# uncertaintyhub/chsimpy

Measured on AMD Instinct MI355X. Metric: timesteps/sec at N=4096 fp64; achieved HBM GB/s vs MI355X peak, higher is better.
Workload: dtype f64; 1 GPU; N=4096 fp64 Cahn-Hilliard timestep loop (BASELINE.json configs[2] at N=4096), U_init = 0.875 + 0.00875*(PCG64(2023).random - 0.5), kappa_tilde=0.0002989112919661156, full_sim; N=4096, engine=fast, ensemble=single run

## Files before the change

### chsimpy_amd/csrc/chs_fast_core.h

```cpp
#pragma once
#include <hip/hip_runtime.h>
#include <type_traits>
#include "chs_cx.h"

template <typename T_, int N_, int G_, int THREADS_, int R0_, int RA_, int RB_, int RL_, int PAD1_, int PAD2_,
          int PADL_, int WPS_, int CT_ = THREADS_ / G_, int XPAIR_ = -1>
struct FCfg {
  using T = T_;
  using V = Cx<T_>;
  static constexpr int N = N_;
  static constexpr int M = N_ / 2;
  static constexpr int G = G_;
  static constexpr int E = M / G_;
  static constexpr int R0 = R0_, RA = RA_, RB = RB_, RL = RL_;
  static constexpr int R2 = RL_;
  static constexpr int S1 = R0_;
  static constexpr int S2A = R0_ * RA_;
  static constexpr int SL = R0_ * RA_ * RB_;
  static constexpr int S2 = SL;
  static constexpr int L1 = M / R0_;
  static constexpr int L2 = L1 / RA_;
  static constexpr int L3 = L2 / RB_;
  static constexpr int NP0 = E / (2 * R0_);
  static constexpr int NBA = E / RA_;
// ... 19 lines not shown
  static_assert(NP0 >= 1 && NP2 >= 1, "E must be >= 2*R0 and >= 2*RL");
  static_assert(RA_ == 1 || NBA >= 1, "E must be >= RA");
  static_assert(RB_ == 1 || NBB >= 1, "E must be >= RB");
  static_assert((G_ <= 64 && (64 % G_) == 0) || (G_ % 64) == 0, "group size");
  static_assert(THREADS_ % G_ == 0 && THREADS_ % 64 == 0, "workgroup size");
};

template <typename T>
struct FTables {
  const T* tw0;
  const T* twa;
  const T* twb;
  const T* wp;
  const T* t1;
  const T* t2;
  const T* lam4;
  const T* sin4;
};

#define FC_SQRT1_2 0.70710678118654752440
#define FC_COS_PI_8 0.92387953251128675613
#define FC_SIN_PI_8 0.38268343236508977173

template <int IDX, bool CONJ>
struct W16 {
  static constexpr int idx = ((CONJ ? -IDX : IDX) % 16 + 16) % 16;
  static constexpr bool pure = (idx % 4) == 0;
};

template <class V, int IDX, bool CONJ>
__device__ __forceinline__ V mul_w16(V a) {
  constexpr int idx = W16<IDX, CONJ>::idx;
  using S = decltype(cx_re(a));
  const V one = cx_make(S(1), S(1));
  if constexpr (idx == 0) {
    return a;
  } else if constexpr (idx == 4) {
    return pk_mul_k<1, 0, 0, 1, 0, 1, 0, 0>(a, one);
  } else if constexpr (idx == 8) {
    return pk_mul_k<0, 1, 0, 1, 1, 1, 0, 0>(a, one);
  } else if constexpr (idx == 12) {
    return pk_mul_k<1, 0, 0, 1, 1, 0, 0, 0>(a, one);
  } else {
    constexpr double cs[16] = {1.0, FC_COS_PI_8, FC_SQRT1_2, FC_SIN_PI_8, 0.0, -FC_SIN_PI_8, -FC_SQRT1_2, -FC_COS_PI_8,
                               -1.0, -FC_COS_PI_8, -FC_SQRT1_2, -FC_SIN_PI_8, 0.0, FC_SIN_PI_8, FC_SQRT1_2, FC_COS_PI_8};
    constexpr double sn[16] = {0.0, FC_SIN_PI_8, FC_SQRT1_2, FC_COS_PI_8, 1.0, FC_COS_PI_8, FC_SQRT1_2, FC_SIN_PI_8,
                               0.0, -FC_SIN_PI_8, -FC_SQRT1_2, -FC_COS_PI_8, -1.0, -FC_COS_PI_8, -FC_SQRT1_2, -FC_SIN_PI_8};
    return cx_mul_k(a, cx_make((S)cs[idx], (S)-sn[idx]));
  }
}

template <class V, int ROT>
__device__ __forceinline__ void bfly2_rot(V& a, V& b) {
  static_assert(ROT % 4 == 0, "pure rotations only");
  constexpr int r = ((ROT % 16) + 16) % 16;
  const V x = a, y = b;
  if constexpr (r == 0) { a = cx_add(x, y); b = cx_sub(x, y); }
  else if constexpr (r == 4) { a = cx_add_mi(x, y); b = cx_add_pi(x, y); }
  else if constexpr (r == 8) { a = cx_sub(x, y); b = cx_add(x, y); }
  else { a = cx_add_pi(x, y); b = cx_add_mi(x, y); }
}

template <class V, int R, bool INV>
struct Dft;

template <class V, bool INV>
struct Dft<V, 1, INV> {
  static __device__ __forceinline__ void run(V*) {}
};

template <class V, bool INV>
struct Dft<V, 2, INV> {
  static __device__ __forceinline__ void run(V* z) { bfly2_rot<V, 0>(z[0], z[1]); }
};

template <class V, bool INV>
struct Dft<V, 4, INV> {
  static __device__ __forceinline__ void run(V* z) {
    const V t0 = cx_add(z[0], z[2]), t1 = cx_sub(z[0], z[2]);
    const V t2 = cx_add(z[1], z[3]), t3 = cx_sub(z[1], z[3]);
    z[0] = cx_add(t0, t2);
    z[2] = cx_sub(t0, t2);
    if constexpr (!INV) { z[1] = cx_add_mi(t1, t3); z[3] = cx_add_pi(t1, t3); }
    else { z[1] = cx_add_pi(t1, t3); z[3] = cx_add_mi(t1, t3); }
  }
};

template <class V, int R, bool INV>
struct Dft {
  static constexpr int A = 4, B = R / 4;
  static_assert(R == 8 || R == 16, "radix must be 2, 4, 8 or 16");
  template <int N2, int K1>
  static constexpr int tw_idx() { return (N2 * K1 * 16) / R; }
  template <int N2, int K1>
  static __device__ __forceinline__ V tw(V a) {
    if constexpr (B == 2 && W16<tw_idx<N2, K1>(), INV>::pure) return a;
    else return mul_w16<V, tw_idx<N2, K1>(), INV>(a);
  }
  template <int N2>
  static __device__ __forceinline__ void col(const V* z, V (*c)[A]) {
    V x[A];
#pragma unroll
    for (int n1 = 0; n1 < A; ++n1) x[n1] = z[B * n1 + N2];
    Dft<V, A, INV>::run(x);
    c[N2][0] = x[0];
    c[N2][1] = tw<N2, 1>(x[1]);
    c[N2][2] = tw<N2, 2>(x[2]);
    c[N2][3] = tw<N2, 3>(x[3]);
  }
  template <int K1>
  static __device__ __forceinline__ void row(V* z, V (*c)[A]) {
    if constexpr (B == 2) {
      V y0 = c[0][K1], y1 = c[1][K1];
      constexpr int rot = W16<tw_idx<1, K1>(), INV>::pure ? W16<tw_idx<1, K1>(), INV>::idx : 0;
      bfly2_rot<V, rot>(y0, y1);
      z[K1] = y0; z[K1 + A] = y1;
    } else {
      V y[B];
#pragma unroll
      for (int n2 = 0; n2 < B; ++n2) y[n2] = c[n2][K1];
      Dft<V, B, INV>::run(y);
#pragma unroll
      for (int k2 = 0; k2 < B; ++k2) z[K1 + A * k2] = y[k2];
    }
  }
  static __device__ __forceinline__ void run(V* z) {
    V c[B][A];
    col<0>(z, c);
    col<1>(z, c);
    if constexpr (B == 4) {
      col<2>(z, c);
      col<3>(z, c);
    }
    row<0>(z, c);
    row<1>(z, c);
    row<2>(z, c);
    row<3>(z, c);
  }
};

template <typename T>
__device__ __forceinline__ Cx<T> ldc(const T* __restrict__ tab, int idx) {
  if constexpr (sizeof(T) == 8) {
    const double2 v = *reinterpret_cast<const double2*>(tab + 2 * (size_t)idx);
    return cx_make(v.x, v.y);
  } else {
    return *reinterpret_cast<const v2f*>(tab + 2 * (size_t)idx);
  }
}

typedef double chs_dv2 __attribute__((ext_vector_type(2)));
template <typename T, bool NT>
__device__ __forceinline__ Cx<T> ldc_hint(const T* __restrict__ tab, int idx) {
  if constexpr (!NT) {
    return ldc<T>(tab, idx);
  } else if constexpr (sizeof(T) == 8) {
    const chs_dv2 v = __builtin_nontemporal_load(reinterpret_cast<const chs_dv2*>(tab + 2 * (size_t)idx));
    return cx_make(v.x, v.y);
  } else {
    return __builtin_nontemporal_load(reinterpret_cast<const v2f*>(tab + 2 * (size_t)idx));
  }
}

template <class C>
__device__ __forceinline__ void xsync() {
  if constexpr (C::WAVE_LOCAL) {
    __builtin_amdgcn_fence(__ATOMIC_RELEASE, "wavefront");
    __builtin_amdgcn_wave_barrier();
    __builtin_amdgcn_fence(__ATOMIC_ACQUIRE, "wavefront");
  } else {
    __syncthreads();
  }
}

// ... 480 lines not shown
```

### chsimpy_amd/csrc/chs_fast_kernels.h

```cpp
#pragma once
#include <cmath>
#include <vector>
#include <cstdlib>

#include "chs_common.h"
#ifdef CHS_STAMPS
#define CHS_NSTAMP 12
#ifdef CHS_FAST_MAIN_TU
__device__ unsigned long long g_stamps[2][8192 * CHS_NSTAMP];
#endif
#define STAMP(K, I)                                                                         \
  do {                                                                                      \
    __builtin_amdgcn_sched_barrier(0);                                                      \
    unsigned long long t__;                                                                 \
    asm volatile("s_memtime %0\n\ts_waitcnt lgkmcnt(0)" : "=s"(t__)::"memory");            \
    __builtin_amdgcn_sched_barrier(0);                                                      \
    if (threadIdx.x == 0 && blockIdx.x < 8192) g_stamps[K][blockIdx.x * CHS_NSTAMP + (I)] = t__; \
  } while (0)
#define CHS_RSTAMP(I) do { if constexpr (PIPE) STAMP(1, 6 + (I)); } while (0)
#define CHS_RSTAMP1(I)                                                                      \
  do {                                                                                      \
    if constexpr (PIPE) {                                                                   \
      __builtin_amdgcn_sched_barrier(0);                                                    \
      unsigned long long t__;                                                               \
// ... 259 lines not shown
  T* ltw = reinterpret_cast<T*>(chs_dyn_lds + (size_t)C::C * C::SCR * sizeof(T) + CHS_LOGTAB_N * 16);
#pragma unroll
  for (int i = 0; i < S::I0; ++i) {
    const int e = 2 * (tid + i * C::THREADS);
    if (e < S::N0) *reinterpret_cast<typename S::Pair*>(ltw + e) = r.a[i];
  }
#pragma unroll
  for (int i = 0; i < S::IM; ++i) {
    const int e = 2 * (tid + i * C::THREADS);
    if (e < S::NM) *reinterpret_cast<typename S::Pair*>(ltw + S::N0 + e) = r.b[i];
  }
  if constexpr (LOGTAB) {
    double2* ltab = reinterpret_cast<double2*>(chs_dyn_lds + (size_t)C::C * C::SCR * sizeof(T));
    if (tid < CHS_LOGTAB_N) ltab[tid] = r.lt;
  }
}
template <class C>
__device__ __forceinline__ FTables<typename C::T> row_tables_in_lds(const FTables<typename C::T>& tb) {
  using S = RowTwSplit<C>;
  using T = typename C::T;
  FTables<T> tbp = tb;
  T* ltw = reinterpret_cast<T*>(chs_dyn_lds + (size_t)C::C * C::SCR * sizeof(T) + CHS_LOGTAB_N * 16);
  if constexpr (S::N0 != 0) tbp.tw0 = ltw;
  tbp.twa = ltw + S::N0;
  tbp.twb = tbp.twa + (C::RA > 1 ? 2 * (C::RA - 1) * C::L2 : 0);
  return tbp;
}

__device__ __forceinline__ int launder(int x) {
  asm volatile("" : "+v"(x));
  __builtin_assume(x >= 0 && x < 1024);
  return x;
}

template <class C, bool POINTWISE>
__global__ __launch_bounds__(C::THREADS, C::WPS) void k_row_fwd(const typename C::T* __restrict__ U, typename C::T* __restrict__ T1,
                                                    FTables<typename C::T> tb, DevConsts dc,
                                                    const DevState* __restrict__ st, double* __restrict__ partMu) {
  using T = typename C::T;
  __shared__ double red[32];
  if (st->halt) return;
  T* lds = reinterpret_cast<T*>(chs_dyn_lds);
  const int wv = chs_wave_id();
  int l, sub;
  row_lane_map<C>(wv, l, sub);
  const int row = row_of_block<C>(blockIdx.x) + sub;
  T* scr = lds + (size_t)sub * C::SCR;
  constexpr int RTWM = RowTwLds<C>::value;
  const FTables<T> tbp = row_twiddles_to_lds<C>(tb, wv * 64 + chs_lane_id());
  if constexpr (RTWM != 0) __syncthreads();
  typename C::V z[C::E];
  double s2 = 0.0;
  const T RT = (T)dc.RT, BRT = (T)dc.BRT, A0 = (T)dc.A0, A1 = (T)dc.A1;
  const unsigned urow = (unsigned)row * C::N;
#pragma unroll
  for (int q = 0; q < C::NP0; ++q) {
    const int m1 = l + C::G * q, m2 = C::L1 - 1 - m1;
#pragma unroll
    for (int j = 0; j < C::R0 / 2; ++j) {
      T q1[4], q2[4];
      load4<T>(at_boff(U, (urow + 4u * (unsigned)(m1 + C::L1 * j)) * (unsigned)sizeof(T)), q1);
      load4<T>(at_boff(U, (urow + 4u * (unsigned)(m2 + C::L1 * j)) * (unsigned)sizeof(T)), q2);
      pack_quads<C>(q1, q2, q, j, z);
    }
  }
  if constexpr (POINTWISE) {
    double2* ltab = reinterpret_cast<double2*>(chs_dyn_lds + (size_t)C::C * C::SCR * sizeof(T));
    if constexpr (sizeof(T) == 8) {
      for (int t = wv * 64 + chs_lane_id(); t < CHS_LOGTAB_N; t += C::THREADS) ltab[t] = reinterpret_cast<const double2*>(chs_log_table)[t];
      __syncthreads();
    }
    unsigned dom = 0;
    auto mu = [&](T& u) {
      const T uinv = T(1) - u;
      const T lU = chs_log_unit_tab<T>(u, ltab, dom), lV = chs_log_unit_tab<T>(uinv, ltab, dom);
      const T m = chs_mu_from_logs_fast<T>(u, uinv, lU, lV, RT, BRT, A0, A1);
      s2 += (double)m * (double)m;
      u = m;
      asm volatile("" : "+v"(u), "+v"(s2), "+v"(dom));
    };
#pragma unroll
    for (int e = 0; e < C::E; ++e) {
      T a = cx_re(z[e]), b = cx_im(z[e]);
      mu(a); mu(b);
      z[e] = cx_make(a, b);
      __builtin_amdgcn_sched_barrier(0);
    }
    if (dom > (unsigned)(CHS_LOGTAB_N - 1)) s2 = __builtin_nan("");
    const double acc1[1] = {s2};
    block_reduce_begin<1, FreshLane<C>::value>(acc1, red, wv);
  }
  fwd_passes<C, (RTWM == 2)>(z, scr, tbp, row_l<C>(wv, l));
  const int lr = row_l<C>(wv, l), sr = row_sub<C>(wv, sub);
  const int rw = row_of_block<C>(blockIdx.x) + sr;
  recombine<C, true, false, false>(z, tb, lr, [](int, const int*) { return NoFetch{}; },
                            [&](int pbase, const int* idx, Cx<T>& Ya, Cx<T>& Yb, bool live, NoFetch) {
    if (live) {
      const T y[4] = {cx_re(Ya), cx_im(Ya), cx_re(Yb), cx_im(Yb)};
      row_store<C>(T1, rw, pbase, launder(lr), idx, y);
    }
  }, [](int, const int*, Cx<T>&, Cx<T>&, bool) {});
  if constexpr (POINTWISE) {
    double tot[1];
    if (block_reduce_end<1, C::THREADS / 64>(red, tot, wv)) partMu[blockIdx.x] = tot[0];
  }
}

template <class C>
__global__ __launch_bounds__(C::THREADS, C::WPS) void k_row_fwd2(const typename C::T* __restrict__ U, typename C::T* __restrict__ Ta,
                                                                 typename C::T* __restrict__ T1, FTables<typename C::T> tb,
                                                                 DevConsts dc, const DevState* __restrict__ st,
                                                                 double* __restrict__ partMu) {
  using T = typename C::T;
  __shared__ double red[32];
  if (st->halt) return;
  T* lds = reinterpret_cast<T*>(chs_dyn_lds);
  const int wv = chs_wave_id();
  int l, sub;
  row_lane_map<C>(wv, l, sub);
  double2* ltab = reinterpret_cast<double2*>(chs_dyn_lds + (size_t)C::C * C::SCR * sizeof(T));
  if constexpr (sizeof(T) == 8) {
    for (int t = wv * 64 + chs_lane_id(); t < CHS_LOGTAB_N; t += C::THREADS) ltab[t] = reinterpret_cast<const double2*>(chs_log_table)[t];
  }
  constexpr int RTWM = RowTwLds<C>::value;
  constexpr bool RTW = (RTWM == 2);
  const FTables<T> tbp = row_twiddles_to_lds<C>(tb, wv * 64 + chs_lane_id());
  if constexpr (sizeof(T) == 8 || RTWM != 0) __syncthreads();
  typename C::V z[C::E];
  const T RT = (T)dc.RT, BRT = (T)dc.BRT, A0 = (T)dc.A0, A1 = (T)dc.A1;
#pragma unroll
  for (int pass = 0; pass < 2; ++pass) {
    const int lp = row_l<C, true>(wv, l);
    const unsigned urow = (unsigned)(row_of_block<C>(blockIdx.x) + row_sub<C, true>(wv, sub)) * C::N;
#pragma unroll
    for (int q = 0; q < C::NP0; ++q) {
      const int m1 = lp + C::G * q, m2 = C::L1 - 1 - m1;
#pragma unroll
      for (int j = 0; j < C::R0 / 2; ++j) {
        T q1[4], q2[4];
        if (pass == 1) {
          load4_nt<T>(at_boff(U, (urow + 4u * (unsigned)(m1 + C::L1 * j)) * (unsigned)sizeof(T)), q1);
          load4_nt<T>(at_boff(U, (urow + 4u * (unsigned)(m2 + C::L1 * j)) * (unsigned)sizeof(T)), q2);
        } else {
          load4<T>(at_boff(U, (urow + 4u * (unsigned)(m1 + C::L1 * j)) * (unsigned)sizeof(T)), q1);
          load4<T>(at_boff(U, (urow + 4u * (unsigned)(m2 + C::L1 * j)) * (unsigned)sizeof(T)), q2);
        }
        pack_quads<C>(q1, q2, q, j, z);
      }
    }
    if (pass == 1) {
      double s2 = 0.0;
      unsigned dom = 0;
      auto mu = [&](T& u) {
        const T uinv = T(1) - u;
        const T lU = chs_log_unit_tab<T>(u, ltab, dom), lV = chs_log_unit_tab<T>(uinv, ltab, dom);
        const T m = chs_mu_from_logs_fast<T>(u, uinv, lU, lV, RT, BRT, A0, A1);
        s2 += (double)m * (double)m;
        u = m;
        asm volatile("" : "+v"(u), "+v"(s2), "+v"(dom));
      };
#pragma unroll
      for (int e = 0; e < C::E; ++e) {
        T a = cx_re(z[e]), b = cx_im(z[e]);
        mu(a); mu(b);
        z[e] = cx_make(a, b);
      }
      if (dom > (unsigned)(CHS_LOGTAB_N - 1)) s2 = __builtin_nan("");
      const double acc1[1] = {s2};
      block_reduce_begin<1, true>(acc1, red, wv);
    }
    T* dst = pass ? T1 : Ta;
    {
      const int lf = row_l<C, true>(wv, l), sf = row_sub<C, true>(wv, sub);
      fwd_passes<C, RTW>(z, lds + (size_t)sf * C::SCR, tbp, lf);
    }
    const int lr = row_l<C, true>(wv, l), sr = row_sub<C, true>(wv, sub);
    const int rw = row_of_block<C>(blockIdx.x) + sr;
    recombine<C, true, false, false>(z, tb, lr, [](int, const int*) { return NoFetch{}; },
                              [&](int pbase, const int* idx, Cx<T>& Ya, Cx<T>& Yb, bool live, NoFetch) {
      if (live) {
        const T y[4] = {cx_re(Ya), cx_im(Ya), cx_re(Yb), cx_im(Yb)};
        if (pass == 0) row_store<C, true>(dst, rw, pbase, launder(lr), idx, y);
        else row_store<C>(dst, rw, pbase, launder(lr), idx, y);
      }
    }, [](int, const int*, Cx<T>&, Cx<T>&, bool) {});
    __builtin_amdgcn_sched_barrier(0);
  }
  double tot[1];
  if (block_reduce_end<1, C::THREADS / 64>(red, tot, wv)) partMu[blockIdx.x] = tot[0];
}

typedef const __attribute__((address_space(4))) BatchMember ConstBatchMember;
template <class P>
__device__ __forceinline__ ConstBatchMember& batch_member(P mem) {
  static_assert(std::is_same<P, const BatchMember*>::value, "batched launches pass the member records");
  return ((ConstBatchMember*)mem)[blockIdx.y];
}

template <class C, bool DIAG, bool FUSE, bool ADAPT = false, class... Batch>
__global__ __launch_bounds__(C::THREADS, C::WPS) void k_row_inv(const typename C::T* __restrict__ T2, typename C::T* __restrict__ U,
                                                    typename C::T* __restrict__ T1, FTables<typename C::T> tb,
                                                    DevConsts dc, const DevState* __restrict__ st,
                                                    double* __restrict__ partDiag, double* __restrict__ partMu,
                                                    double* __restrict__ partRa, int store_u,
                                                    typename C::T* __restrict__ partColRows = nullptr, Batch... mem) {
  using T = typename C::T;
  __shared__ double red[64];
  if constexpr (sizeof...(Batch) != 0) {
    static_assert(DIAG && (FUSE || !ADAPT), "batches run the step's row kernels");
    ConstBatchMember& m = batch_member(mem...);
    const long long done = m.st->rows_written, last = m.nsteps - 1;
    if (FUSE ? done >= last : done != last) return;
    T2 = (const T*)m.T2; U = (T*)m.U; T1 = (T*)m.T1; dc = *(const DevConsts*)&m.dc; st = m.st;
    partDiag = m.partDiag; partMu = m.partMu; partRa = m.partRa;
    if constexpr (ADAPT) partColRows = (T*)m.partColRows;
  }
  if (st->halt) return;
  T* lds = reinterpret_cast<T*>(chs_dyn_lds);
  const int wv = chs_wave_id();
  int l, sub;
// ... 41 lines not shown
#pragma unroll
    for (int q = 0; q < C::NP0; ++q) {
      const int m1 = ls + C::G * q, m2 = C::L1 - 1 - m1;
#pragma unroll
      for (int j = 0; j < C::R0 / 2; ++j) {
        T q1[4], q2[4];
        unpack_quads<C>(z, q, j, q1, q2);
        T* p1 = at_boff(U, (urow + 4u * (unsigned)(m1 + C::L1 * j)) * (unsigned)sizeof(T));
        T* p2 = at_boff(U, (urow + 4u * (unsigned)(m2 + C::L1 * j)) * (unsigned)sizeof(T));
        if constexpr (decltype(nt)::value) { store4_nt<T>(p1, q1); store4_nt<T>(p2, q2); }
        else { store4<T>(p1, q1); store4<T>(p2, q2); }
      }
    }
  };
  if (FUSE && store_u) put_u(std::true_type{});
  else if (write_u) put_u(std::false_type{});
  if constexpr (DIAG) {
    if (ls == 0) {
      T q1[4], q2[4];
      unpack_quads<C>(z, 0, 0, q1, q2);
      const double d0 = (double)q1[1] - (double)q1[0];
      unpack_quads<C>(z, 0, C::R0 / 2 - 1, q1, q2);
      const double d1 = (double)q2[3] - (double)q2[2];
      sEdge += d0 * d0 + d1 * d1;
    }
  }
  if constexpr (DIAG && FUSE) STAMP(0, 3);
  __builtin_amdgcn_sched_barrier(0);
  if constexpr (DIAG) {
    constexpr int RR = C::N / 2 + 1;
    const bool ra_blk = (row0 == (RR / C::C) * C::C);
    if (ra_blk) {
      const bool mine = ra_blk && row_sub<C>(wv, sub) == RR % C::C;
      double rs = 0.0;
      if (mine) {
#pragma unroll
        for (int e = 0; e < C::E; ++e) rs += (double)cx_re(z[e]) + (double)cx_im(z[e]);
      }
      const double rmean = block_sum_w(rs, red, wv, C::THREADS / 64) / (double)C::N;
      double ad = 0.0;
      if (mine) {
#pragma unroll
        for (int e = 0; e < C::E; ++e) ad += fabs((double)cx_re(z[e]) - rmean) + fabs((double)cx_im(z[e]) - rmean);
      }
      const double ra = block_sum_w(ad, red, wv, C::THREADS / 64) / (double)C::N;
      if (ra_blk && wv == 0 && chs_lane_id() == 0) partRa[0] = ra;
      __syncthreads();
    }
    const T RT = (T)dc.RT, BRT = (T)dc.BRT, B = (T)dc.B, A0 = (T)dc.A0, A1 = (T)dc.A1;
    const double mean = mean_u, thr = dc.threshold;
    double sE = 0.0, sPS = 0.0, s2 = 0.0;
    int cSA = 0;
    unsigned dom = 0;
    auto point = [&](T& u) {
      const T uinv = T(1) - u;
      const T lU = chs_log_unit_tab<T>(u, ltab, dom), lV = chs_log_unit_tab<T>(uinv, ltab, dom);
      sE += (double)chs_energy_from_logs_fast<T>(u, uinv, lU, lV, RT, B, A0, A1);
      sPS += fabs((double)u - mean);
      cSA += ((double)u < thr) ? 1 : 0;
      if constexpr (FUSE) {
        const T m = chs_mu_from_logs_fast<T>(u, uinv, lU, lV, RT, BRT, A0, A1);
        s2 += (double)m * (double)m;
        u = m;
        asm volatile("" : "+v"(u), "+v"(s2));
      }
      asm volatile("" : "+v"(sE), "+v"(sPS), "+v"(cSA), "+v"(dom));
    };
#pragma unroll
    for (int e = 0; e < C::E; ++e) {
      T a = cx_re(z[e]), b = cx_im(z[e]);
      point(a);
      point(b);
      z[e] = cx_make(a, b);
      __builtin_amdgcn_sched_barrier(0);
    }
    if (dom > (unsigned)(CHS_LOGTAB_N - 1)) sE = __builtin_nan("");
    const double acc[5] = {sE, sEdge, sPS, (double)cSA, s2};
    block_reduce_begin<5, FreshLane<C>::value>(acc, red, wv);
  }
  if constexpr (ADAPT) {
    constexpr int LDSB = C::C * C::SCR * (int)sizeof(T);
    constexpr int NH = (C::C == 1 || C::N * (int)sizeof(T) <= LDSB) ? 1 : 2;
    constexpr int JH = (C::R0 / 2) / NH;
    static_assert(!ADAPT || (FUSE && C::C <= 4 && (C::C == 1 || C::N * (int)sizeof(T) / NH <= LDSB) && (C::R0 / 2) % NH == 0),
                  "partial column sums need the scratch");
    const long long cs = st->computed_steps + 1;
    if (cs > 500 && (cs % 2) == 0) {
      const int lg = row_l<C>(wv, l);
      const int sub_a = row_sub<C>(wv, sub);
      T* prow = partColRows + (size_t)blockIdx.x * C::N;
      T* gl = reinterpret_cast<T*>(chs_dyn_lds);
      const T dmax = (T)dc.delt_max;
#pragma unroll
      for (int h = 0; h < NH; ++h) {
#pragma unroll
        for (int s = C::C - 1; s >= 0; --s) {
          __syncthreads();
          if (sub_a == s) {
#pragma unroll
            for (int q = 0; q < C::NP0; ++q) {
              const int m1 = lg + C::G * q, m2 = C::L1 - 1 - m1;
#pragma unroll
              for (int j = h * JH; j < (h + 1) * JH; ++j) {
                T q1[4], q2[4];
                unpack_quads<C>(z, q, j, q1, q2);
                const int c1 = 4 * (m1 + C::L1 * j), c2 = 4 * (m2 + C::L1 * j);
                const int o1 = c1 - h * (C::N / NH), o2 = c2 - h * (C::N / NH);
                T g1[4], g2[4];
#pragma unroll
                for (int e = 0; e < 4; ++e) {
                  g1[e] = chs_dt_integrand_fast(q1[e], dmax);
                  g2[e] = chs_dt_integrand_fast(q2[e], dmax);
                  if (s < C::C - 1) { g1[e] += gl[o1 + e]; g2[e] += gl[o2 + e]; }
                  if (s > 0) { gl[o1 + e] = g1[e]; gl[o2 + e] = g2[e]; }
                }
                if (s == 0) {
                  if constexpr (chs_grid_exceeds_cache(C::N, sizeof(T))) { store4_nt<T>(&prow[c1], g1); store4_nt<T>(&prow[c2], g2); }
                  else { store4<T>(&prow[c1], g1); store4<T>(&prow[c2], g2); }
                }
                __builtin_amdgcn_sched_barrier(0);
              }
            }
          }
        }
      }
      __syncthreads();
    }
  }
  if constexpr (DIAG && FUSE) STAMP(0, 4);
// ... 631 lines not shown
```

### chsimpy_amd/csrc/chs_math.h

```cpp
#pragma once
#include <hip/hip_runtime.h>
#include "chs_common.h"

#define CHS_LN2_HI 0.6931471803691238
#define CHS_LN2_LO 1.9082149292705877e-10
#define CHS_SQRT2 1.4142135623730951
#define CHS_SQRT1_2 0.7071067811865476

__device__ __forceinline__ double chs_div_pos(double d, double sig) {
  double r = __builtin_amdgcn_rcp(sig);
  double e = __builtin_fma(-sig, r, 1.0);
  r = __builtin_fma(r, e, r);
  e = __builtin_fma(-sig, r, 1.0);
  r = __builtin_fma(r, e, r);
  double q = d * r;
  const double rho = __builtin_fma(-sig, q, d);
  return __builtin_fma(rho, r, q);
}

__device__ __forceinline__ double chs_div_pos1(double d, double sig) {
  double r = __builtin_amdgcn_rcp(sig);
  const double e = __builtin_fma(-sig, r, 1.0);
  r = __builtin_fma(r, e, r);
  const double q = d * r;
// ... 11 lines not shown
  p = __builtin_fma(p, z, 0.3999999999987206);
  p = __builtin_fma(p, z, 0.6666666666666671);
  return __builtin_fma(s * z, p, s + s);
}

__device__ __forceinline__ double chs_log_f64(double x) {
  double m = __builtin_amdgcn_frexp_mant(x);
  int e = __builtin_amdgcn_frexp_exp(x);
  const int c = (m < CHS_SQRT1_2) ? 1 : 0;
  m = __builtin_ldexp(m, c);
  e -= c;
  const double s = chs_div_pos(m - 1.0, m + 1.0);
  const double lq = chs_log_poly(s);
  const double k = (double)e;
  double res = __builtin_fma(k, CHS_LN2_HI, __builtin_fma(k, CHS_LN2_LO, lq));
  asm volatile("" : "+v"(res));
  const double bad = (x == 0.0) ? -__builtin_inf() : __builtin_nan("");
  res = (x > 0.0) ? res : bad;
  res = (x == __builtin_inf()) ? x : res;
  return res;
}

__device__ __forceinline__ double chs_log_pos_f64(double x) {
  double m = __builtin_amdgcn_frexp_mant(x);
  int e = __builtin_amdgcn_frexp_exp(x);
  const int c = (m < CHS_SQRT1_2) ? 1 : 0;
  m = __builtin_ldexp(m, c);
  e -= c;
  const double s = chs_div_pos1(m - 1.0, m + 1.0);
  const double lq = chs_log_poly(s);
  const double k = (double)e;
  return __builtin_fma(k, CHS_LN2_HI, __builtin_fma(k, CHS_LN2_LO, lq));
}

__device__ __forceinline__ double chs_log_ratio_f64(double a, double b) {
  double ma = __builtin_amdgcn_frexp_mant(a), mb = __builtin_amdgcn_frexp_mant(b);
  const int ea = __builtin_amdgcn_frexp_exp(a), eb = __builtin_amdgcn_frexp_exp(b);
  const int c1 = (ma > CHS_SQRT2 * mb) ? 1 : 0;
  const int c2 = (CHS_SQRT2 * ma < mb) ? 1 : 0;
  mb = __builtin_ldexp(mb, c1);
  ma = __builtin_ldexp(ma, c2);
  const int e = ea - eb + c1 - c2;
  const double s = chs_div_pos(ma - mb, ma + mb);
  const double lq = chs_log_poly(s);
  const double k = (double)e;
  double res = __builtin_fma(k, CHS_LN2_HI, __builtin_fma(k, CHS_LN2_LO, lq));
  asm volatile("" : "+v"(res));
  const bool ok = (a > 0.0) && (b > 0.0) && (a < __builtin_inf()) && (b < __builtin_inf());
  return ok ? res : __builtin_nan("");
}

#include "chs_log_table.h"
#define CHS_LN2 0.6931471805599453
__device__ __forceinline__ double chs_log_unit_tab_f64(double x, const double2* tab, unsigned& domain) {
#pragma clang fp contract(off)
  const double m = __builtin_amdgcn_frexp_mant(x);
  const int e = __builtin_amdgcn_frexp_exp(x);
  const double u = __builtin_fma(m, 256.0, 0x1.8p52);
  const unsigned i = (unsigned)(__double2loint(u) - CHS_LOGTAB_I0);
  domain = max(domain, i);
  const double2 t = tab[min(i, (unsigned)(CHS_LOGTAB_N - 1))];
  const double r = __builtin_fma(m, t.x, -1.0);
  double p = __builtin_fma(r, -1.0 / 6.0, 1.0 / 5.0);
  p = __builtin_fma(r, p, -1.0 / 4.0);
  p = __builtin_fma(r, p, 1.0 / 3.0);
  p = __builtin_fma(r, p, -0.5);
  const double lp = __builtin_fma(r * r, p, r);
  return __builtin_fma((double)e, CHS_LN2, t.y) + lp;
}

__device__ __forceinline__ float chs_logf(float x) {
  return __builtin_amdgcn_logf(x) * 0.69314718055994530942f;
}
template <typename T> __device__ __forceinline__ T chs_log_pos(T x);
template <> __device__ __forceinline__ double chs_log_pos<double>(double x) { return chs_log_pos_f64(x); }
template <> __device__ __forceinline__ float chs_log_pos<float>(float x) { return chs_logf(x); }
template <typename T> __device__ __forceinline__ T chs_log_unit_tab(T x, const double2* tab, unsigned& domain);
template <> __device__ __forceinline__ double chs_log_unit_tab<double>(double x, const double2* tab, unsigned& domain) { return chs_log_unit_tab_f64(x, tab, domain); }
template <> __device__ __forceinline__ float chs_log_unit_tab<float>(float x, const double2*, unsigned& domain) {
  domain = max(domain, (x > 0.0f) ? 0u : ~0u);
  return chs_logf(x);
}

template <typename T> __device__ __forceinline__ T chs_log(T x);
template <> __device__ __forceinline__ double chs_log<double>(double x) { return chs_log_f64(x); }
template <> __device__ __forceinline__ float chs_log<float>(float x) { return chs_logf(x); }

template <typename T> __device__ __forceinline__ T chs_log_ratio(T a, T b);
template <> __device__ __forceinline__ double chs_log_ratio<double>(double a, double b) { return chs_log_ratio_f64(a, b); }
template <> __device__ __forceinline__ float chs_log_ratio<float>(float a, float b) { return chs_logf(a / b); }

template <typename T>
__device__ __forceinline__ T chs_mu(T U, T RT, T BRT, T A0, T A1) {
#pragma clang fp contract(off)
  const T Uinv = T(1) - U;
  const T U2inv = Uinv - U;
  const T t1 = RT * chs_log_ratio<T>(U, Uinv);
  const T t2 = (A0 + A1 * U2inv) * U2inv;
  const T t3 = ((T(2) * A1) * U) * Uinv;
  return ((t1 - BRT) + t2) - t3;
}

template <typename T>
__device__ __forceinline__ T chs_energy_density(T U, T RT, T B, T A0, T A1) {
#pragma clang fp contract(off)
  const T Uinv = T(1) - U;
  const T a = U * (chs_log<T>(U) - B);
  const T b = Uinv * chs_log<T>(Uinv);
  const T c = ((A0 + A1 * (Uinv - U)) * U) * Uinv;
  return RT * (a + b) + c;
}

template <typename T>
__device__ __forceinline__ T chs_energy_from_logs(T U, T Uinv, T lU, T lV, T RT, T B, T A0, T A1) {
#pragma clang fp contract(off)
  const T a = U * (lU - B);
  const T b = Uinv * lV;
  const T c = ((A0 + A1 * (Uinv - U)) * U) * Uinv;
  return RT * (a + b) + c;
}
template <typename T>
__device__ __forceinline__ T chs_mu_from_logs(T U, T Uinv, T lU, T lV, T RT, T BRT, T A0, T A1) {
#pragma clang fp contract(off)
  const T U2inv = Uinv - U;
  const T t1 = RT * (lU - lV);
  const T t2 = (A0 + A1 * U2inv) * U2inv;
  const T t3 = ((T(2) * A1) * U) * Uinv;
  return ((t1 - BRT) + t2) - t3;
}

template <typename T>
__device__ __forceinline__ T chs_energy_from_logs_fast(T U, T Uinv, T lU, T lV, T RT, T B, T A0, T A1) {
  const T a = U * (lU - B);
  const T b = Uinv * lV;
  const T c = ((A0 + A1 * (Uinv - U)) * U) * Uinv;
  return RT * (a + b) + c;
}
template <typename T>
__device__ __forceinline__ T chs_mu_from_logs_fast(T U, T Uinv, T lU, T lV, T RT, T BRT, T A0, T A1) {
  const T U2inv = Uinv - U;
  const T t1 = RT * (lU - lV);
  const T t2 = (A0 + A1 * U2inv) * U2inv;
  const T t3 = ((T(2) * A1) * U) * Uinv;
  return ((t1 - BRT) + t2) - t3;
}

__device__ __forceinline__ double chs_dt_integrand(double mu, double delt_max) {
#pragma clang fp contract(off)
  const double a = 62.5 * (mu * mu);
  return delt_max / sqrt(1.0 + a);
}

__device__ __forceinline__ double chs_dt_integrand_fast(double mu, double delt_max) {
  const double a = __builtin_fma(62.5 * mu, mu, 1.0);
  const double h = 0.5 * a;
  double y = __builtin_amdgcn_rsq(a);
  y = y * __builtin_fma(-h * y, y, 1.5);
  y = y * __builtin_fma(-h * y, y, 1.5);
  return delt_max * y;
}
__device__ __forceinline__ float chs_dt_integrand_fast(float mu, float delt_max) {
  return delt_max * __builtin_amdgcn_rsqf(__builtin_fmaf(62.5f * mu, mu, 1.0f));
}

#ifndef CHS_F32_SPECTRAL_MIN_N
#define CHS_F32_SPECTRAL_MIN_N 8192
#endif
__device__ __forceinline__ float chs_spectral_f32(float hatU, float hatMu, double li, double lj, double lam1, double lam2) {
  const float leig = (float)li + (float)lj;
  const float CHeig = __builtin_fmaf((float)lam2 * leig, leig, 1.0f);
  const float rhs = __builtin_fmaf((float)lam1 * leig, hatMu, hatU);
  const float r = __builtin_amdgcn_rcpf(CHeig);
  const float q = rhs * r;
  const float rho = __builtin_fmaf(-CHeig, q, rhs);
  return __builtin_fmaf(rho, r, q);
}
template <typename T, bool F32MATH = false>
__device__ __forceinline__ T chs_spectral(T hatU, T hatMu, double li, double lj, double lam1, double lam2) {
#pragma clang fp contract(off)
  if constexpr (sizeof(T) == 4 && F32MATH) return chs_spectral_f32(hatU, hatMu, li, lj, lam1, lam2);
  const double leig = li + lj;
  const double CHeig = 1.0 + (lam2 * leig) * leig;
  const double Seig = lam1 * leig;
  const double rhs = (double)hatU + Seig * (double)hatMu;
  return (T)chs_div_pos1(rhs, CHeig);
}
```

### chsimpy_amd/csrc/chs_pointwise.hip

```cpp
#include "chs_common.h"
#include "chs_math.h"
#include "chs_tail.h"
#include "chs_nat_batch.h"

#define PW_THREADS 256
#define DISPATCH_T(E, expr_d, expr_f) \
  do { if ((E)->dtype == CHS_F64) { expr_d; } else { expr_f; } } while (0)
#define PW_BAND 8
#define DIAG_BAND 32

template <typename T, class... Batch>
__global__ __launch_bounds__(PW_THREADS) void k_mu(const T* __restrict__ U, T* __restrict__ MU, DevConsts dc,
                                                   const DevState* __restrict__ st, double* __restrict__ partMu,
                                                   double* __restrict__ partCol, int only_col, int cs_offset, Batch... sel) {
  __shared__ double scratch[32];
  if constexpr (sizeof...(Batch) != 0) {
    ConstNatMember& m = nat_member(NatSel{sel...}, blockIdx.y);
    if (nat_sits_out(m)) return;
    U = (const T*)m.arr[NAT_U]; MU = (T*)m.arr[NAT_MU]; dc = *(const DevConsts*)&m.dc; st = m.st; partMu = m.partMu;
  } else {
    if (st->halt) return;
  }
  const int N = dc.N;
  const int r0 = blockIdx.x * PW_BAND;
// ... 108 lines not shown
                                                     const DevState* __restrict__ st,
                                                     double* __restrict__ partDiag, int ignore_halt, Batch... sel) {
  __shared__ double scratch[32];
  __shared__ double2 ltab[CHS_LOGTAB_N];
  if constexpr (sizeof...(Batch) != 0) {
    ConstNatMember& m = nat_member(NatSel{sel...}, blockIdx.z);
    if (nat_sits_out(m)) return;
    U = (const T*)m.arr[NAT_U]; dc = *(const DevConsts*)&m.dc; st = m.st; partDiag = m.partDiag;
  } else {
    if (!ignore_halt && st->halt) return;
  }
  if constexpr (sizeof(T) == 8) {
    for (int t = threadIdx.x; t < CHS_LOGTAB_N; t += PW_THREADS) ltab[t] = reinterpret_cast<const double2*>(chs_log_table)[t];
    __syncthreads();
  }
  const int N = dc.N;
  const int r0 = blockIdx.x * DIAG_BAND, r1 = min(r0 + DIAG_BAND, N);
  const int c = blockIdx.y * PW_THREADS + threadIdx.x;
  const double mean = st->meanU;
  const double inv2dx = 1.0 / (2.0 * dc.delx), invdx = 1.0 / dc.delx;
  const T RT = (T)dc.RT, B = (T)dc.B, A0 = (T)dc.A0, A1 = (T)dc.A1;
  double sE = 0.0, sG = 0.0, sPS = 0.0, cSA = 0.0;
  unsigned dom = 0;
  if (c < N) {
    const T* col = U + c;
    T up = r0 > 0 ? col[(size_t)(r0 - 1) * N] : T(0), cur = col[(size_t)r0 * N];
    for (int r = r0; r < r1; ++r) {
      const size_t o = (size_t)r * N;
      const T nxt = r < N - 1 ? col[o + N] : T(0);
      const T lft = c > 0 ? col[o - 1] : T(0), rgt = c < N - 1 ? col[o + 1] : T(0);
      const double ud = (double)cur;
      double gx, gy;
      if (r == 0)
        gx = ((double)nxt - ud) * invdx;
      else if (r == N - 1)
        gx = (ud - (double)up) * invdx;
      else
        gx = ((double)nxt - (double)up) * inv2dx;
      if (c == 0)
        gy = ((double)rgt - ud) * invdx;
      else if (c == N - 1)
        gy = (ud - (double)lft) * invdx;
      else
        gy = ((double)rgt - (double)lft) * inv2dx;
      sG += gx * gx + gy * gy;
      const T uinv = T(1) - cur;
      const T lU = chs_log_unit_tab<T>(cur, ltab, dom), lV = chs_log_unit_tab<T>(uinv, ltab, dom);
      sE += (double)chs_energy_from_logs<T>(cur, uinv, lU, lV, RT, B, A0, A1);
      sPS += fabs(ud - mean);
      cSA += (ud < dc.threshold) ? 1.0 : 0.0;
      up = cur; cur = nxt;
    }
  }
  if (dom > (unsigned)(CHS_LOGTAB_N - 1)) sE = __builtin_nan("");
  const double tE = block_sum(sE, scratch);
  const double tG = block_sum(sG, scratch);
  const double tP = block_sum(sPS, scratch);
  const double tS = block_sum(cSA, scratch);
  if (threadIdx.x == 0) {
    double* p = partDiag + ((size_t)blockIdx.y * gridDim.x + blockIdx.x) * 4;
    p[0] = tE; p[1] = tG; p[2] = tP; p[3] = tS;
  }
}


template <typename T, class... Batch>
__global__ __launch_bounds__(PW_THREADS) void k_fin(const T* __restrict__ U, DevConsts dc, DevState* __restrict__ st,
                                                    const double* __restrict__ partDiag, int nPart,
                                                    double* __restrict__ rows, long long rowsCap, int prepare_mode,
                                                    const double* __restrict__ partE2, int nE2, int fused, Batch... sel) {
  __shared__ double scratch[32];
  if constexpr (sizeof...(Batch) != 0) {
    ConstNatMember& m = nat_member(NatSel{sel...}, blockIdx.x);
    if (nat_sits_out(m)) return;
    U = (const T*)m.arr[NAT_U]; dc = *(const DevConsts*)&m.dc; st = m.st; partDiag = m.partDiag;
    rows = m.rows; rowsCap = m.rowsCap;
  } else {
    if (!prepare_mode && st->halt) return;
  }
  const int N = dc.N;
  double sE = 0.0, sG = 0.0, sP = 0.0, sS = 0.0;
  for (int i = threadIdx.x; i < nPart; i += PW_THREADS) {
    sE += partDiag[(size_t)i * 4 + 0];
    sG += partDiag[(size_t)i * 4 + 1];
    sP += partDiag[(size_t)i * 4 + 2];
    sS += partDiag[(size_t)i * 4 + 3];
  }
  sE = block_sum(sE, scratch);
  sG = block_sum(sG, scratch);
  sP = block_sum(sP, scratch);
  sS = block_sum(sS, scratch);
  if (fused) {
    double sp = 0.0;
    for (int i = threadIdx.x; i < nE2; i += PW_THREADS) sp += partE2[i];
    sp = block_sum(sp, scratch);
    double er = 0.0;
    for (int c = threadIdx.x; c < N; c += PW_THREADS) {
      const double d0 = (double)U[(size_t)N + c] - (double)U[c];
      const double d1 = (double)U[(size_t)(N - 1) * N + c] - (double)U[(size_t)(N - 2) * N + c];
      er += d0 * d0 + d1 * d1;
    }
    er = block_sum(er, scratch);
    sG = (4.0 * sp + 3.0 * (sG + er)) / (4.0 * dc.delx * dc.delx);
  }
  const int rr = N / 2 + 1;
  double s = 0.0;
  if (rr < N)
// ... 500 lines not shown
  if (blocks > 4096) blocks = 4096;
  const dim3 grid(blocks, B);
  const NatSel sel{mem, NAT_T2, NAT_HAT};
  DISPATCH_T(E0,
    (k_spectral<double, NatSel><<<grid, PW_THREADS, 0, s>>>(nullptr, nullptr, E0->dLambda, E0->N, nullptr, sel)),
    (k_spectral<float, NatSel><<<grid, PW_THREADS, 0, s>>>(nullptr, nullptr, E0->dLambda, E0->N, nullptr, sel)));
  CHS_HIP(hipGetLastError());
  return CHS_OK;
}

int chs_nat_batch_diag(Engine* E0, hipStream_t s, const NatMember* mem, int B) {
  const dim3 grid((E0->N + DIAG_BAND - 1) / DIAG_BAND, (E0->N + PW_THREADS - 1) / PW_THREADS, B);
  const NatSel sel{mem, NAT_U, NAT_U};
  DISPATCH_T(E0,
    (k_diag<double, NatSel><<<grid, PW_THREADS, 0, s>>>(nullptr, E0->dc, nullptr, nullptr, 0, sel)),
    (k_diag<float, NatSel><<<grid, PW_THREADS, 0, s>>>(nullptr, E0->dc, nullptr, nullptr, 0, sel)));
  CHS_HIP(hipGetLastError());
  return CHS_OK;
}

int chs_nat_batch_fin(Engine* E0, hipStream_t s, const NatMember* mem, int B) {
  const NatSel sel{mem, NAT_U, NAT_U};
  DISPATCH_T(E0,
    (k_fin<double, NatSel><<<B, PW_THREADS, 0, s>>>(nullptr, E0->dc, nullptr, nullptr, E0->nDiagBlocks, nullptr, 0, 0, nullptr, 0, 0, sel)),
    (k_fin<float, NatSel><<<B, PW_THREADS, 0, s>>>(nullptr, E0->dc, nullptr, nullptr, E0->nDiagBlocks, nullptr, 0, 0, nullptr, 0, 0, sel)));
  CHS_HIP(hipGetLastError());
  return CHS_OK;
}

int chs_launch_jitter(Engine* E) {
  const size_t total = (size_t)E->N * E->N;
  const int blocks = jitter_blocks(total);
  chs_slot_begin(E, SLOT_MISC);
  DISPATCH_T(E,
    (k_jitter<double><<<blocks, PW_THREADS, 0, E->stream>>>((double*)E->dU, (const double*)E->dNoise, E->jitter, total,
                                                             E->dState, E->dPartSum)),
    (k_jitter<float><<<blocks, PW_THREADS, 0, E->stream>>>((float*)E->dU, (const float*)E->dNoise, E->jitter, total,
                                                            E->dState, E->dPartSum)));
  k_sum_fin<<<1, PW_THREADS, 0, E->stream>>>(E->dPartSum, blocks, E->N, E->dState, 0);
  chs_slot_end(E, SLOT_MISC);
  CHS_HIP(hipGetLastError());
  return CHS_OK;
}

__global__ void k_test_math(int which, const double* __restrict__ a, const double* __restrict__ b,
                            double* __restrict__ out, long long n) {
  __shared__ double2 ltab[CHS_LOGTAB_N];
  for (int t = threadIdx.x; t < CHS_LOGTAB_N; t += blockDim.x) ltab[t] = reinterpret_cast<const double2*>(chs_log_table)[t];
  __syncthreads();
  const long long i = (long long)blockIdx.x * blockDim.x + threadIdx.x;
  if (i >= n) return;
  double r;
  unsigned dom = 0;
  if (which == 5) { r = chs_log_unit_tab_f64(a[i], ltab, dom); if (dom > (unsigned)(CHS_LOGTAB_N - 1)) r = __builtin_nan(""); }
  else if (which == 0) r = chs_log_f64(a[i]);
  else if (which == 1) r = chs_log_ratio_f64(a[i], b[i]);
  else if (which == 4) r = chs_log_pos_f64(a[i]);
  else if (which == 2) r = chs_mu<double>(a[i], b[0], b[1], b[2], b[3]);
  else r = chs_energy_density<double>(a[i], b[0], b[1], b[2], b[3]);
  out[i] = r;
}

extern "C" int chs_test_math(int device, int which, const double* a, const double* b, double* out, int64_t n) {
  if (!a || !out || n <= 0 || which < 0 || which > 5) { chs_set_error("chs_test_math: bad argument"); return CHS_EINVAL; }
  CHS_HIP(hipSetDevice(device));
  double *da = nullptr, *db = nullptr, *dout = nullptr;
  const size_t nb_b = (which == 1) ? (size_t)n : 4;
  CHS_HIP(hipMalloc(&da, sizeof(double) * n));
  CHS_HIP(hipMalloc(&db, sizeof(double) * nb_b));
  CHS_HIP(hipMalloc(&dout, sizeof(double) * n));
  CHS_HIP(hipMemcpy(da, a, sizeof(double) * n, hipMemcpyHostToDevice));
  if (b) CHS_HIP(hipMemcpy(db, b, sizeof(double) * nb_b, hipMemcpyHostToDevice));
  k_test_math<<<(unsigned)((n + 255) / 256), 256>>>(which, da, db, dout, (long long)n);
  CHS_HIP(hipGetLastError());
  CHS_HIP(hipDeviceSynchronize());
  CHS_HIP(hipMemcpy(out, dout, sizeof(double) * n, hipMemcpyDeviceToHost));
  hipFree(da); hipFree(db); hipFree(dout);
  return CHS_OK;
}
```

Before: 4801 timesteps/s.

## Fold FFT twiddles into radix-4 butterflies and fuse fp64 energy/mu arithmetic

```diff
diff --git a/chsimpy_amd/csrc/chs_fast_core.h b/chsimpy_amd/csrc/chs_fast_core.h
--- a/chsimpy_amd/csrc/chs_fast_core.h
+++ b/chsimpy_amd/csrc/chs_fast_core.h
@@ -95,13 +95,37 @@
 
 template <class V, int ROT>
 __device__ __forceinline__ void bfly2_rot(V& a, V& b) {
-  static_assert(ROT % 4 == 0, "pure rotations only");
+  static_assert(ROT % 2 == 0, "roots of equal-magnitude components only");
   constexpr int r = ((ROT % 16) + 16) % 16;
   const V x = a, y = b;
   if constexpr (r == 0) { a = cx_add(x, y); b = cx_sub(x, y); }
   else if constexpr (r == 4) { a = cx_add_mi(x, y); b = cx_add_pi(x, y); }
   else if constexpr (r == 8) { a = cx_sub(x, y); b = cx_add(x, y); }
-  else { a = cx_add_pi(x, y); b = cx_add_mi(x, y); }
+  else if constexpr (r == 12) { a = cx_add_pi(x, y); b = cx_add_mi(x, y); }
+  else {
+    using S = decltype(cx_re(a));
+    const V k = cx_make((S)FC_SQRT1_2, (S)FC_SQRT1_2);
+    const V uv = cx_add_mi(y, y);
+    if constexpr (r == 2)       { a = pk_fma_k<0, 1, 0, 1, 0, 0, 0, 0>(uv, k, x); b = pk_fma_k<0, 1, 0, 1, 1, 1, 0, 0>(uv, k, x); }
+    else if constexpr (r == 6)  { a = pk_fma_k<1, 0, 0, 1, 0, 1, 0, 0>(uv, k, x); b = pk_fma_k<1, 0, 0, 1, 1, 0, 0, 0>(uv, k, x); }
+    else if constexpr (r == 10) { a = pk_fma_k<0, 1, 0, 1, 1, 1, 0, 0>(uv, k, x); b = pk_fma_k<0, 1, 0, 1, 0, 0, 0, 0>(uv, k, x); }
+    else                        { a = pk_fma_k<1, 0, 0, 1, 1, 0, 0, 0>(uv, k, x); b = pk_fma_k<1, 0, 0, 1, 0, 1, 0, 0>(uv, k, x); }
+  }
+}
+
+template <class V, int R1, int R2, int R3, int ROTI>
+__device__ __forceinline__ void dft4_rot(V* y) {
+  constexpr bool F2 = (R2 % 2) == 0;
+  constexpr bool F13 = (R1 % 4) == 2 && ((R3 - R1) % 16 + 16) % 4 == 0;
+  V t0 = y[0], t1 = y[2], t2 = y[1], t3 = y[3];
+  if constexpr (F2) bfly2_rot<V, R2>(t0, t1);
+  else { t1 = mul_w16<V, R2, false>(t1); bfly2_rot<V, 0>(t0, t1); }
+  if constexpr (F13) bfly2_rot<V, R3 - R1>(t2, t3);
+  else { t2 = mul_w16<V, R1, false>(t2); t3 = mul_w16<V, R3, false>(t3); bfly2_rot<V, 0>(t2, t3); }
+  constexpr int P = F13 ? R1 : 0;
+  bfly2_rot<V, P>(t0, t2);
+  bfly2_rot<V, P + ROTI>(t1, t3);
+  y[0] = t0; y[2] = t2; y[1] = t1; y[3] = t3;
 }
 
 template <class V, int R, bool INV>
@@ -136,33 +160,27 @@
   template <int N2, int K1>
   static constexpr int tw_idx() { return (N2 * K1 * 16) / R; }
   template <int N2, int K1>
-  static __device__ __forceinline__ V tw(V a) {
-    if constexpr (B == 2 && W16<tw_idx<N2, K1>(), INV>::pure) return a;
-    else return mul_w16<V, tw_idx<N2, K1>(), INV>(a);
-  }
+  static constexpr int rot() { return W16<tw_idx<N2, K1>(), INV>::idx; }
   template <int N2>
   static __device__ __forceinline__ void col(const V* z, V (*c)[A]) {
     V x[A];
 #pragma unroll
     for (int n1 = 0; n1 < A; ++n1) x[n1] = z[B * n1 + N2];
     Dft<V, A, INV>::run(x);
-    c[N2][0] = x[0];
-    c[N2][1] = tw<N2, 1>(x[1]);
-    c[N2][2] = tw<N2, 2>(x[2]);
-    c[N2][3] = tw<N2, 3>(x[3]);
+#pragma unroll
+    for (int k1 = 0; k1 < A; ++k1) c[N2][k1] = x[k1];
   }
   template <int K1>
   static __device__ __forceinline__ void row(V* z, V (*c)[A]) {
     if constexpr (B == 2) {
       V y0 = c[0][K1], y1 = c[1][K1];
-      constexpr int rot = W16<tw_idx<1, K1>(), INV>::pure ? W16<tw_idx<1, K1>(), INV>::idx : 0;
-      bfly2_rot<V, rot>(y0, y1);
+      bfly2_rot<V, rot<1, K1>()>(y0, y1);
       z[K1] = y0; z[K1 + A] = y1;
     } else {
       V y[B];
 #pragma unroll
       for (int n2 = 0; n2 < B; ++n2) y[n2] = c[n2][K1];
-      Dft<V, B, INV>::run(y);
+      dft4_rot<V, rot<1, K1>(), rot<2, K1>(), rot<3, K1>(), INV ? 12 : 4>(y);
 #pragma unroll
       for (int k2 = 0; k2 < B; ++k2) z[K1 + A * k2] = y[k2];
     }
diff --git a/chsimpy_amd/csrc/chs_fast_kernels.h b/chsimpy_amd/csrc/chs_fast_kernels.h
--- a/chsimpy_amd/csrc/chs_fast_kernels.h
+++ b/chsimpy_amd/csrc/chs_fast_kernels.h
@@ -335,6 +335,7 @@
   typename C::V z[C::E];
   double s2 = 0.0;
   const T RT = (T)dc.RT, BRT = (T)dc.BRT, A0 = (T)dc.A0, A1 = (T)dc.A1;
+  [[maybe_unused]] const PwConsts pwk = chs_pw_consts(dc.RT, dc.B, dc.BRT, dc.A0, dc.A1);
   const unsigned urow = (unsigned)row * C::N;
 #pragma unroll
   for (int q = 0; q < C::NP0; ++q) {
@@ -357,7 +358,9 @@
     auto mu = [&](T& u) {
       const T uinv = T(1) - u;
       const T lU = chs_log_unit_tab<T>(u, ltab, dom), lV = chs_log_unit_tab<T>(uinv, ltab, dom);
-      const T m = chs_mu_from_logs_fast<T>(u, uinv, lU, lV, RT, BRT, A0, A1);
+      T m;
+      if constexpr (sizeof(T) == 8) { T e; chs_energy_mu_from_logs<false, true>(u, uinv, lU, lV, pwk, e, m); }
+      else m = chs_mu_from_logs_fast<T>(u, uinv, lU, lV, RT, BRT, A0, A1);
       s2 += (double)m * (double)m;
       u = m;
       asm volatile("" : "+v"(u), "+v"(s2), "+v"(dom));
@@ -369,7 +372,7 @@
       z[e] = cx_make(a, b);
       __builtin_amdgcn_sched_barrier(0);
     }
-    if (dom > (unsigned)(CHS_LOGTAB_N - 1)) s2 = __builtin_nan("");
+    if (chs_log_dom_bad(dom)) s2 = __builtin_nan("");
     const double acc1[1] = {s2};
     block_reduce_begin<1, FreshLane<C>::value>(acc1, red, wv);
   }
@@ -411,6 +414,7 @@
   if constexpr (sizeof(T) == 8 || RTWM != 0) __syncthreads();
   typename C::V z[C::E];
   const T RT = (T)dc.RT, BRT = (T)dc.BRT, A0 = (T)dc.A0, A1 = (T)dc.A1;
+  [[maybe_unused]] const PwConsts pwk = chs_pw_consts(dc.RT, dc.B, dc.BRT, dc.A0, dc.A1);
 #pragma unroll
   for (int pass = 0; pass < 2; ++pass) {
     const int lp = row_l<C, true>(wv, l);
@@ -437,7 +441,9 @@
       auto mu = [&](T& u) {
         const T uinv = T(1) - u;
         const T lU = chs_log_unit_tab<T>(u, ltab, dom), lV = chs_log_unit_tab<T>(uinv, ltab, dom);
-        const T m = chs_mu_from_logs_fast<T>(u, uinv, lU, lV, RT, BRT, A0, A1);
+        T m;
+        if constexpr (sizeof(T) == 8) { T e; chs_energy_mu_from_logs<false, true>(u, uinv, lU, lV, pwk, e, m); }
+        else m = chs_mu_from_logs_fast<T>(u, uinv, lU, lV, RT, BRT, A0, A1);
         s2 += (double)m * (double)m;
         u = m;
         asm volatile("" : "+v"(u), "+v"(s2), "+v"(dom));
@@ -448,7 +454,7 @@
         mu(a); mu(b);
         z[e] = cx_make(a, b);
       }
-      if (dom > (unsigned)(CHS_LOGTAB_N - 1)) s2 = __builtin_nan("");
+      if (chs_log_dom_bad(dom)) s2 = __builtin_nan("");
       const double acc1[1] = {s2};
       block_reduce_begin<1, true>(acc1, red, wv);
     }
@@ -596,14 +602,20 @@
     double sE = 0.0, sPS = 0.0, s2 = 0.0;
     int cSA = 0;
     unsigned dom = 0;
+    [[maybe_unused]] const PwConsts pwk = chs_pw_consts(dc.RT, dc.B, dc.BRT, dc.A0, dc.A1);
     auto point = [&](T& u) {
       const T uinv = T(1) - u;
       const T lU = chs_log_unit_tab<T>(u, ltab, dom), lV = chs_log_unit_tab<T>(uinv, ltab, dom);
-      sE += (double)chs_energy_from_logs_fast<T>(u, uinv, lU, lV, RT, B, A0, A1);
+      [[maybe_unused]] T m = T(0);
+      if constexpr (sizeof(T) == 8) {
+        chs_energy_mu_from_logs<true, FUSE>(u, uinv, lU, lV, pwk, sE, m);
+      } else {
+        sE += (double)chs_energy_from_logs_fast<T>(u, uinv, lU, lV, RT, B, A0, A1);
+        if constexpr (FUSE) m = chs_mu_from_logs_fast<T>(u, uinv, lU, lV, RT, BRT, A0, A1);
+      }
       sPS += fabs((double)u - mean);
       cSA += ((double)u < thr) ? 1 : 0;
       if constexpr (FUSE) {
-        const T m = chs_mu_from_logs_fast<T>(u, uinv, lU, lV, RT, BRT, A0, A1);
         s2 += (double)m * (double)m;
         u = m;
         asm volatile("" : "+v"(u), "+v"(s2));
@@ -618,7 +630,7 @@
       z[e] = cx_make(a, b);
       __builtin_amdgcn_sched_barrier(0);
     }
-    if (dom > (unsigned)(CHS_LOGTAB_N - 1)) sE = __builtin_nan("");
+    if (chs_log_dom_bad(dom)) sE = __builtin_nan("");
     const double acc[5] = {sE, sEdge, sPS, (double)cSA, s2};
     block_reduce_begin<5, FreshLane<C>::value>(acc, red, wv);
   }
diff --git a/chsimpy_amd/csrc/chs_math.h b/chsimpy_amd/csrc/chs_math.h
--- a/chsimpy_amd/csrc/chs_math.h
+++ b/chsimpy_amd/csrc/chs_math.h
@@ -87,22 +87,24 @@
 
 #include "chs_log_table.h"
 #define CHS_LN2 0.6931471805599453
+#define CHS_LOG_DOM_MAX 0x100FFFu
+__device__ __forceinline__ bool chs_log_dom_bad(unsigned domain) { return domain > CHS_LOG_DOM_MAX; }
 __device__ __forceinline__ double chs_log_unit_tab_f64(double x, const double2* tab, unsigned& domain) {
 #pragma clang fp contract(off)
   const double m = __builtin_amdgcn_frexp_mant(x);
   const int e = __builtin_amdgcn_frexp_exp(x);
-  const double u = __builtin_fma(m, 256.0, 0x1.8p52);
-  const unsigned i = (unsigned)(__double2loint(u) - CHS_LOGTAB_I0);
-  domain = max(domain, i);
-  const double2 t = tab[min(i, (unsigned)(CHS_LOGTAB_N - 1))];
+  const unsigned w = (unsigned)__double2hiint(m) - (0x3FE00000u - 0x1000u);
+  domain = max(domain, w);
+  const double2 t = tab[min(w, CHS_LOG_DOM_MAX) >> 13];
   const double r = __builtin_fma(m, t.x, -1.0);
   double p = __builtin_fma(r, -1.0 / 6.0, 1.0 / 5.0);
   p = __builtin_fma(r, p, -1.0 / 4.0);
   p = __builtin_fma(r, p, 1.0 / 3.0);
   p = __builtin_fma(r, p, -0.5);
-  const double lp = __builtin_fma(r * r, p, r);
-  return __builtin_fma((double)e, CHS_LN2, t.y) + lp;
-}
+  const double q = __builtin_fma(r, p, 1.0);
+  return __builtin_fma(r, q, __builtin_fma((double)e, CHS_LN2, t.y));
+}
+static_assert((CHS_LOG_DOM_MAX >> 13) == CHS_LOGTAB_N - 1, "the clamped index is the table's last entry");
 
 __device__ __forceinline__ float chs_logf(float x) {
   return __builtin_amdgcn_logf(x) * 0.69314718055994530942f;
@@ -178,6 +180,33 @@
   const T t2 = (A0 + A1 * U2inv) * U2inv;
   const T t3 = ((T(2) * A1) * U) * Uinv;
   return ((t1 - BRT) + t2) - t3;
+}
+
+struct PwConsts {
+  double RT, A0, A1, A1h, nRTB, c0;
+};
+__device__ __forceinline__ PwConsts chs_pw_consts(double RT, double B, double BRT, double A0, double A1) {
+  PwConsts k;
+  k.RT = RT; k.A0 = A0; k.A1 = A1; k.A1h = 1.5 * A1; k.nRTB = -(RT * B); k.c0 = -(BRT + 0.5 * A1);
+  return k;
+}
+template <bool ENERGY, bool MU>
+__device__ __forceinline__ void chs_energy_mu_from_logs(double U, double Uinv, double lU, double lV, const PwConsts& k,
+                                                        double& sE, double& mu) {
+  const double V2 = Uinv - U;
+  const double d = lU - lV;
+  if constexpr (ENERGY) {
+    const double g = __builtin_fma(k.A1, V2, k.A0);
+    const double t = __builtin_fma(g, Uinv, k.nRTB);
+    const double s = __builtin_fma(U, d, lV);
+    sE = __builtin_fma(k.RT, s, sE);
+    sE = __builtin_fma(U, t, sE);
+  }
+  if constexpr (MU) {
+    const double h = __builtin_fma(k.A1h, V2, k.A0);
+    const double m = __builtin_fma(k.RT, d, k.c0);
+    mu = __builtin_fma(V2, h, m);
+  }
 }
 
 __device__ __forceinline__ double chs_dt_integrand(double mu, double delt_max) {
diff --git a/chsimpy_amd/csrc/chs_pointwise.hip b/chsimpy_amd/csrc/chs_pointwise.hip
--- a/chsimpy_amd/csrc/chs_pointwise.hip
+++ b/chsimpy_amd/csrc/chs_pointwise.hip
@@ -184,7 +184,7 @@
       up = cur; cur = nxt;
     }
   }
-  if (dom > (unsigned)(CHS_LOGTAB_N - 1)) sE = __builtin_nan("");
+  if (chs_log_dom_bad(dom)) sE = __builtin_nan("");
   const double tE = block_sum(sE, scratch);
   const double tG = block_sum(sG, scratch);
   const double tP = block_sum(sPS, scratch);
@@ -791,7 +791,7 @@
   if (i >= n) return;
   double r;
   unsigned dom = 0;
-  if (which == 5) { r = chs_log_unit_tab_f64(a[i], ltab, dom); if (dom > (unsigned)(CHS_LOGTAB_N - 1)) r = __builtin_nan(""); }
+  if (which == 5) { r = chs_log_unit_tab_f64(a[i], ltab, dom); if (chs_log_dom_bad(dom)) r = __builtin_nan(""); }
   else if (which == 0) r = chs_log_f64(a[i]);
   else if (which == 1) r = chs_log_ratio_f64(a[i], b[i]);
   else if (which == 4) r = chs_log_pos_f64(a[i]);
```

After: 4926 timesteps/s (median of 6 runs). 2.6% higher.
